# Kaz-K/medical-image-editing

Hardware: AMD Instinct MI355X
Metric: images/sec (train step, 256x256 2D slices) (higher is better)
Workload: dtype f32

## Files before the change

### medical-image-editing_amd/csrc/conv_wino64.hip

```cpp
#include "common.h"
#include "conv_common.h"
#include "mfma_util.h"
#include "wino_common.h"

extern int g_wino_mode;

namespace {

struct W64Args {
    const float* x;
    const float* u;
    const float* bias;
    float* y;
    int N, H, W, Cin, Cout;
    int tilesY, tilesX, nsp;
    int ntn, nch;
    int kt;
    int relu;
    unsigned nbx, nbu, nby;
    float* stats;
    const float* mask;
    const float* mr;
    int in_relu;
    float* y2;
    int split, pool0;
    int c1;
    unsigned nby2;
    unsigned img_px, rowb_px, rpx, ppx;
    int n_sh, n_m;
};

constexpr int W6_KPH = wino::KPH;
template <int RW, int MBW, int NW = 8> struct W64Geo {
    static_assert(MBW == 1 || (MBW == 2 && RW == 32), "two M blocks per wave: 32-wide regions only");
    static_assert(NW == 8 || (NW == 4 && RW == 32), "four-wave workgroups: 32-wide regions only");
    static constexpr int NMB = NW / 2;
    static constexpr int NBW = 4 / MBW;
    static constexpr int NCO = 16 * NBW;
    static constexpr int TR = RW == 32 ? 2 * MBW * NMB : 16;
    static constexpr int HR = TR + 2, HWV = RW + 2;
    static constexpr int HWS = RW == 32 ? 34 : 24;
    static constexpr int HBUF = HR * HWS * W6_KPH;
    static constexpr int UBUF = 16 * NCO * 8;
    static constexpr int EXF = 2048 * NW;
    static_assert(EXF >= UBUF, "U buffer 1 lives in the exchange area");
    static constexpr size_t LDS_FLOATS = 2 * HBUF + UBUF + EXF + 2 * NMB * NCO * 2;
};
constexpr int W6_LS = 4;
constexpr int W6_CP = 26;
constexpr int W6_CP1 = 26;
constexpr int W6_PB = 33, W6_CB = 58;

template <int RW, int MBW, int EPI, int NW = 8>
__global__ void __launch_bounds__(64 * NW, 8 / NW) k_conv_wino64(W64Args a) {
    constexpr bool MASK = EPI >= 1 && EPI <= 3;
    using G = W64Geo<RW, MBW, NW>;
    constexpr int NT = 64 * NW, NMB = G::NMB, NBW = G::NBW, NCO = G::NCO;
    constexpr int HWS = G::HWS, HWV = G::HWV, HBUF = G::HBUF, UBUF = G::UBUF;
    using Halo = wino::HaloStager<NT, G::HR, HWV, HWS, wino::PitchedPix>;
    constexpr int LH = Halo::LH;
    constexpr int LU = 512 * NBW / NT;
    constexpr int CP = MBW == 1 ? W6_CP1 : W6_CP;
    constexpr int CPMAX = MBW == 1 ? 64 : 32;
    constexpr bool ONE_PHASE = 1 + (LH + LU) * W6_LS <= CP && CP + LH + LU <= CPMAX;
    constexpr int LUA = ONE_PHASE ? LU : LU / 2;
    static_assert(1 + (LH + LUA) * W6_LS <= CP && CP + LH + LUA <= CPMAX, "prefetch slots fit the first half of an item");
    static_assert(ONE_PHASE || (LU == 2 * LUA && W6_PB + LUA * W6_LS <= W6_CB && W6_CB + LUA <= 64), "second U phase fits the second half");

    extern __shared__ __attribute__((aligned(16))) float smem[];
    float* Hs = smem;
    float* Us = smem + 2 * HBUF;
    float* Ex = Us + UBUF;
    float* Rs = Ex + G::EXF;

    const int tid = threadIdx.x, lane = tid & 63;
    const int wv = __builtin_amdgcn_readfirstlane(tid >> 6);
    const int mb = wv & (NMB - 1), h = wv / NMB;
    const int H = a.H, W = a.W, Cin = a.Cin, Cout = a.Cout;
    const __amdgpu_buffer_rsrc_t rsx = make_rsrc(a.x, a.nbx), rsu = make_rsrc(a.u, a.nbu), rsy = make_rsrc(a.y, a.nby);
    const __amdgpu_buffer_rsrc_t rsm = make_rsrc((EPI == 1 || EPI == 3) ? a.mask : a.y, a.nby);
    const __amdgpu_buffer_rsrc_t rsr = make_rsrc(EPI == 3 ? a.mr : a.y, EPI == 3 ? (unsigned)((size_t)a.N * a.Cout * 8) : a.nby);
    const __amdgpu_buffer_rsrc_t rsy2 = make_rsrc(EPI == 4 ? a.y2 : a.y, EPI == 4 ? a.nby2 : a.nby);

    const int nch = a.nch;
    const wino::RegionRun run = wino::region_run(a.ntn, a.kt, a.nsp);
    const int co_base = run.tile_n * NCO;
    const int my_tiles = run.my_tiles;
    if (my_tiles <= 0) return;

    const int c4 = tid & 1;
    const wino::PitchedPix pixel = {a.img_px, a.rowb_px, a.rpx, a.ppx, a.n_sh, a.n_m};
    Halo hs;
    hs.init(tid, pixel);
    auto region_offsets = [&](int n, int tx, int ty) { hs.region_offsets(n, ty * G::TR - 1, tx * RW - 1, H, W, Cin); };
    const int u_n = (tid >> 1) & (NCO - 1);
    const unsigned u_voff = (((unsigned)(tid >> 1) / NCO * Cout + co_base + u_n) * 8u + c4 * 4) * 4u;
    const unsigned u_jstride = (unsigned)(NT / 2 / NCO) * Cout * 32u;
    const unsigned u_cstride = 16u * Cout * 32u;
    const int u_lds = (tid >> 1) * 8 + ((c4 ^ ((u_n >> 3) & 1)) * 4);

    float4 ru[LUA];
    auto issue_h = [&](int j, int chunk) { hs.issue_h(rsx, j, chunk); };
    auto commit_h = [&](int j, float* Hb) { hs.commit_h(j, Hb); };
    auto issue_u = [&](int j, int chunk) {
        u32x4 v = __builtin_amdgcn_raw_buffer_load_b128(rsu, (int)u_voff, (int)(chunk * u_cstride + j * u_jstride), 0);
        unsigned a0 = v[0], a1 = v[1], a2 = v[2], a3 = v[3];
        float4& r = ru[j % LUA];
        r.x = __uint_as_float(a0); r.y = __uint_as_float(a1); r.z = __uint_as_float(a2); r.w = __uint_as_float(a3);
    };
    auto commit_u = [&](int j, float* Ub) { *(float4*)&Ub[u_lds + j * (NT * 4)] = ru[j % LUA]; };

    int cn, ctx, cty, ch = 0;
    region_start(run.sp0, a.tilesY, a.tilesX, cn, ctx, cty);
    auto advance = [&](int& n, int& tx, int& ty, int& c) {
        const int adv = c + 1 == nch ? 1 : 0;
        c = adv ? 0 : c + 1;
        region_step(adv, a.tilesY, a.tilesX, n, tx, ty);
    };
    int n1 = cn, tx1 = ctx, ty1 = cty, ch1 = 0;
    advance(n1, tx1, ty1, ch1);
    int n2 = n1, tx2 = tx1, ty2 = ty1, ch2 = ch1;
    advance(n2, tx2, ty2, ch2);
    auto shift = [&]() {
        cn = n1; ctx = tx1; cty = ty1; ch = ch1;
        n1 = n2; tx1 = tx2; ty1 = ty2; ch1 = ch2;
        advance(n2, tx2, ty2, ch2);
    };

    const int m = lane & 15, q = lane >> 4;
    const int rA = h ? 3 : 0, rB = h ? 2 : 1, rC = h ? 1 : 2;
    const int prow = RW == 32 ? 2 * MBW * mb : 2 * (2 * mb + (m >> 3)), pcol = RW == 32 ? 2 * m : 2 * (m & 7);
    constexpr int MBW_STEP = 2 * HWS * W6_KPH;
    const int a_A = opaque(((prow + rA) * HWS + pcol) * W6_KPH + 2 * q);
    const int a_B = opaque(((prow + rB) * HWS + pcol) * W6_KPH + 2 * q);
    const int a_C = opaque(((prow + rC) * HWS + pcol) * W6_KPH + 2 * q);
    const int b_swz = ((q >> 1) ^ (m >> 3)) * 4 + (q & 1) * 2;
    const int b_0 = opaque(((h ? 3 : 0) * 4 * NCO + m) * 8 + b_swz);
    const int b_1 = opaque(((h ? 2 : 1) * 4 * NCO + m) * 8 + b_swz);
    const float sg = opaque_f(h ? -1.f : 1.f), mone = opaque_f(-1.f);

    f32x4 acc[8][MBW][NBW];
    f32x2 bf[2][NBW];
    f32x2 dcol[2][3];
    float e[2][2][4];
    float v[2][MBW][2][8];

    auto read_col = [&](const float* Hb, int w, int c) {
        const float* Hc = Hb + w * MBW_STEP + c * W6_KPH;
        dcol[c & 1][0] = *(const f32x2*)&Hc[a_A];
        dcol[c & 1][1] = *(const f32x2*)&Hc[a_B];
        dcol[c & 1][2] = *(const f32x2*)&Hc[a_C];
    };
    auto xform_op = [&](int par, int w, int o) {
        if (o < 16) {
            const int c = o >> 2, k = o & 3, t = k >> 1;
            const float dA = dcol[c & 1][0][t], dB = dcol[c & 1][1][t], dC = dcol[c & 1][2][t];
            if ((k & 1) == 0) e[t][0][c] = __builtin_fmaf(mone, dC, dA);
            else e[t][1][c] = __builtin_fmaf(sg, dC, dB);
        } else {
            const int k = o - 16, lr = k >> 3, t = (k >> 2) & 1, cc = k & 3;
            const float e0 = e[t][lr][0], e1 = e[t][lr][1], e2 = e[t][lr][2], e3 = e[t][lr][3];
            v[par][w][t][lr * 4 + cc] = wino::bt_row_plain(cc, e0, e1, e2, e3);
        }
    };
    auto xform_slot = [&](const float* Hn, int par, int p) {
        constexpr int NOPS = 32 * MBW, P0 = MBW == 1 ? 32 : 4;
        auto op = [&](int g) { xform_op(par, g >> 5, g & 31); };
        auto rd = [&](int g) {
            if ((g & 31) < 16 && ((g & 31) & 3) == 0) read_col(Hn, g >> 5, (g & 31) >> 2);
        };
        if (p + 3 - P0 >= 0 && p + 3 - P0 < NOPS) rd(p + 3 - P0);
        if (p - P0 >= 0 && p - P0 < NOPS && p < 64) {
            const int g = p - P0;
            if (P0 + NOPS <= 64 || g < NOPS - 2 * (P0 + NOPS - 64)) op(g);
            else { const int d = g - (NOPS - 2 * (P0 + NOPS - 64)); op(NOPS - 2 * (P0 + NOPS - 64) + 2 * d); op(NOPS - 2 * (P0 + NOPS - 64) + 2 * d + 1); }
        }
    };

    region_offsets(cn, ctx, cty);
#pragma unroll
    for (int j = 0; j < LH; ++j) issue_h(j, 0);
#pragma unroll
    for (int j = 0; j < LUA; ++j) issue_u(j, 0);
#pragma unroll
    for (int j = 0; j < LH; ++j) commit_h(j, Hs);
#pragma unroll
    for (int j = 0; j < LUA; ++j) commit_u(j, Us);
#pragma unroll
    for (int j = LUA; j < LU; ++j) issue_u(j, 0);
#pragma unroll
    for (int j = LUA; j < LU; ++j) commit_u(j, Us);
    region_offsets(n1, tx1, ty1);
#pragma unroll
    for (int j = 0; j < LH; ++j) issue_h(j, ch1);
#pragma unroll
    for (int j = 0; j < LH; ++j) commit_h(j, Hs + HBUF);
    __syncthreads();
#pragma unroll
    for (int w = 0; w < MBW; ++w)
#pragma unroll
        for (int o = 0; o < 32; ++o) {
            if (o < 16 && (o & 3) == 0) read_col(Hs, w, o >> 2);
            xform_op(0, w, o);
        }
    __syncthreads();
    region_offsets(n2, tx2, ty2);

    float bvv[NBW / 2];
#pragma unroll
    for (int i = 0; i < NBW / 2; ++i) bvv[i] = a.bias ? a.bias[co_base + (h * (NBW / 2) + i) * 16 + m] : 0.f;
    const float lo = a.relu ? 0.f : -__builtin_inff();
    const bool plain = a.bias == nullptr && !a.relu;
    int spar = 0;

    auto body = [&](auto PAR, auto FIRST) {
        constexpr int par = decltype(PAR)::value;
        constexpr bool first = decltype(FIRST)::value;
        const float* Uc = Us + par * UBUF;
        const float* Hn = Hs + (par ^ 1) * HBUF;
        float* Hw = Hs + par * HBUF;
        float* Uw = Us + (par ^ 1) * UBUF;
        auto ldb = [&](int l, int nb) {
            bf[l & 1][nb] = *(const f32x2*)&Uc[(l < 4 ? b_0 : b_1) + ((l & 3) * NCO + nb * 16) * 8];
        };
        auto slot = [&](int p) {
            if (p >= 1 && p < 1 + LH * W6_LS && (p - 1) % W6_LS == 0) issue_h((p - 1) / W6_LS, ch2);
            if (p >= CP && p < CP + LH) commit_h(p - CP, Hw);
            if (p >= 1 + LH * W6_LS && p < 1 + (LH + LUA) * W6_LS && (p - 1) % W6_LS == 0) issue_u((p - 1) / W6_LS - LH, ch1);
            if (p >= CP + LH && p < CP + LH + LUA) commit_u(p - CP - LH, Uw);
            if (!ONE_PHASE) {
                if (p >= W6_PB && p < W6_PB + LUA * W6_LS && (p - W6_PB) % W6_LS == 0) issue_u(LUA + (p - W6_PB) / W6_LS, ch1);
                if (p >= W6_CB && p < W6_CB + LUA) commit_u(LUA + p - W6_CB, Uw);
            }
            xform_slot(Hn, par ^ 1, p);
        };
#pragma unroll
        for (int nb = 0; nb < NBW; ++nb) { ldb(0, nb); __builtin_amdgcn_sched_barrier(0); }
        const f32x4 zero4 = {0.f, 0.f, 0.f, 0.f};
        if (first) {
#pragma unroll
            for (int p = 0; p < 8; ++p) slot(p);
#pragma unroll
            for (int w = 0; w < MBW; ++w)
#pragma unroll
                for (int nb = 0; nb < NBW; ++nb) acc[7][w][nb] = zero4;
        } else {
#pragma unroll
            for (int j = 0; j < 8; ++j) {
                const int w = j / (2 * NBW), k = (j / NBW) & 1, nb = j % NBW;
                acc[7][w][nb] = MFMA16(v[par ^ 1][w][k][7], k == 0 ? bf[1][nb].x : bf[1][nb].y, acc[7][w][nb]);
                slot(j);
                __builtin_amdgcn_sched_barrier(0);
            }
        }
#pragma unroll
        for (int l = 0; l < 7; ++l) {
#pragma unroll
            for (int j = 0; j < 8; ++j) {
                const int w = j / (2 * NBW), k = (j / NBW) & 1, nb = j % NBW;
                if (j < NBW) ldb(l + 1, nb);
                acc[l][w][nb] = MFMA16(v[par][w][k][l], k == 0 ? bf[l & 1][nb].x : bf[l & 1][nb].y, (first && k == 0) ? zero4 : acc[l][w][nb]);
                slot(8 + l * 8 + j);
                __builtin_amdgcn_sched_barrier(0);
            }
        }
    };
    auto flush = [&]() {
#pragma unroll
        for (int j = 0; j < 8; ++j) {
            const int w = j / (2 * NBW), k = (j / NBW) & 1, nb = j % NBW;
            acc[7][w][nb] = MFMA16(v[1][w][k][7], k == 0 ? bf[1][nb].x : bf[1][nb].y, acc[7][w][nb]);
            __builtin_amdgcn_sched_barrier(0);
        }
    };

    auto partial = [&](auto HH, int w, int nb, int r, float* yv) {
        constexpr int hh = decltype(HH)::value;
        float p0[4], p1[4];
#pragma unroll
        for (int j = 0; j < 4; ++j) {
            const float l0 = acc[j][w][nb][r], l1 = acc[4 + j][w][nb][r];
            if (hh == 0) { p0[j] = l0 + l1; p1[j] = l1; }
            else { p0[j] = l1; p1[j] = l0 - l1; }
        }
        yv[0] = (p0[0] + p0[1]) + p0[2];
        yv[1] = (p0[1] - p0[2]) - p0[3];
        yv[2] = (p1[0] + p1[1]) + p1[2];
        yv[3] = (p1[1] - p1[2]) - p1[3];
    };
    auto epi_send = [&](auto HH) {
        constexpr int hh = decltype(HH)::value;
        float* Xo = Ex + (((mb * 2 + (hh ^ 1)) * 8) * 64 + lane) * 4;
#pragma unroll
        for (int w = 0; w < MBW; ++w)
#pragma unroll
            for (int i = 0; i < NBW / 2; ++i)
#pragma unroll
                for (int r = 0; r < 4; ++r) {
                    float yv[4];
                    partial(HH, w, (hh ^ 1) * (NBW / 2) + i, r, yv);
                    float4 o;
                    o.x = yv[0]; o.y = yv[1]; o.z = yv[2]; o.w = yv[3];
                    *(float4*)&Xo[((w * (NBW / 2) + i) * 4 + r) * 256] = o;
                }
    };
    auto epi_finish = [&](auto HH) {
        constexpr int hh = decltype(HH)::value;
        const float* Xi = Ex + (((mb * 2 + hh) * 8) * 64 + lane) * 4;
        float st1[NBW / 2], st2[NBW / 2];
#pragma unroll
        for (int w = 0; w < MBW; ++w) {
            const int yrow0 = cty * G::TR + (RW == 32 ? 2 * (MBW * mb + w) : 2 * (2 * mb + (q >> 1)));
            const int xcol0 = ctx * RW + (RW == 32 ? 8 * q : 8 * (q & 1));
#pragma unroll
            for (int i = 0; i < NBW / 2; ++i) {
                float yv[16];
                const int co0 = co_base + (hh * (NBW / 2) + i) * 16;
                const unsigned co = (unsigned)(co0 + m);
                const bool part0 = EPI == 4 && co0 < a.split;
                const bool pooled = part0 && a.pool0;
                const unsigned cs = EPI != 4 ? (unsigned)Cout : (unsigned)(part0 ? a.split : a.c1);
                const unsigned cc = EPI != 4 ? co : (part0 ? co : co - (unsigned)a.split);
                int voffs[2];
#pragma unroll
                for (int aa = 0; aa < 2; ++aa) {
                    const int yy = yrow0 + aa;
                    const unsigned base = (pixel.base(cn) + (unsigned)yy * a.rpx + (unsigned)xcol0 * a.ppx) * cs + cc;
                    voffs[aa] = (int)sel_u32(yy < H, base * 4u, 0xFFFFFFFFu);
                }
                float mk[16];
                if (MASK) {
#pragma unroll
                    for (int aa = 0; aa < 2; ++aa)
#pragma unroll
                        for (int r = 0; r < 4; ++r)
#pragma unroll
                            for (int b = 0; b < 2; ++b)
                                mk[r * 4 + aa * 2 + b] = __uint_as_float(__builtin_amdgcn_raw_buffer_load_b32(rsm, voffs[aa], (2 * r + b) * (int)a.ppx * Cout * 4, 0));
                }
#pragma unroll
                for (int r = 0; r < 4; ++r) {
                    float own[4];
                    partial(HH, w, hh * (NBW / 2) + i, r, own);
                    const float4 o = *(const float4*)&Xi[((w * (NBW / 2) + i) * 4 + r) * 256];
                    if (plain) {
                        yv[r * 4 + 0] = own[0] + o.x; yv[r * 4 + 1] = own[1] + o.y;
                        yv[r * 4 + 2] = own[2] + o.z; yv[r * 4 + 3] = own[3] + o.w;
                    } else {
                        yv[r * 4 + 0] = fmaxf((own[0] + o.x) + bvv[i], lo);
                        yv[r * 4 + 1] = fmaxf((own[1] + o.y) + bvv[i], lo);
                        yv[r * 4 + 2] = fmaxf((own[2] + o.z) + bvv[i], lo);
                        yv[r * 4 + 3] = fmaxf((own[3] + o.w) + bvv[i], lo);
                    }
                }
                if (EPI == 1) {
#pragma unroll
                    for (int k = 0; k < 16; ++k) yv[k] = mk[k] > 0.f ? yv[k] : 0.f;
                } else if (EPI == 2) {
#pragma unroll
                    for (int k = 0; k < 16; ++k) yv[k] = mk[k] + yv[k];
                } else if (EPI == 3) {
                    const unsigned mo = ((unsigned)(cn >> a.n_sh) * (unsigned)Cout + co) * 8u;
                    const float mean = __uint_as_float(__builtin_amdgcn_raw_buffer_load_b32(rsr, (int)mo, 0, 0));
                    const float rstd = __uint_as_float(__builtin_amdgcn_raw_buffer_load_b32(rsr, (int)mo, 4, 0));
                    float s1 = 0.f, s2 = 0.f;
#pragma unroll
                    for (int k = 0; k < 16; ++k) {
                        const float xh = (mk[k] - mean) * rstd;
                        const float gm = (a.in_relu && !(xh > 0.f)) ? 0.f : yv[k];
                        s1 += gm;
                        s2 = __builtin_fmaf(gm, xh, s2);
                    }
                    s1 += __shfl_xor(s1, 16, 64); s2 += __shfl_xor(s2, 16, 64);
                    s1 += __shfl_xor(s1, 32, 64); s2 += __shfl_xor(s2, 32, 64);
                    if (w == 0) { st1[i] = s1; st2[i] = s2; }
                    else { st1[i] += s1; st2[i] += s2; }
                }
                if (EPI == 4 && !part0 && co0 - a.split >= a.c1) {
                } else if (EPI == 4 && pooled) {
                    const unsigned base = (((unsigned)cn * (unsigned)(H >> 1) + (unsigned)(yrow0 >> 1)) * (unsigned)(W >> 1) + (unsigned)(xcol0 >> 1)) * cs + cc;
                    const int voff = (int)sel_u32(yrow0 < H, base * 4u, 0xFFFFFFFFu);
#pragma unroll
                    for (int r = 0; r < 4; ++r) {
                        const float t = (yv[r * 4 + 0] + yv[r * 4 + 1]) + (yv[r * 4 + 2] + yv[r * 4 + 3]);
                        __builtin_amdgcn_raw_buffer_store_b32(__float_as_uint(t), rsy, voff, r * (int)cs * 4, 0);
                    }
                } else {
#pragma unroll
                    for (int aa = 0; aa < 2; ++aa) {
                        const int voff = voffs[aa];
#pragma unroll
                        for (int r = 0; r < 4; ++r)
#pragma unroll
                            for (int b = 0; b < 2; ++b)
                                __builtin_amdgcn_raw_buffer_store_b32(__float_as_uint(yv[r * 4 + aa * 2 + b]), (EPI == 4 && !part0) ? rsy2 : rsy, voff,
                                                                      (2 * r + b) * (int)(a.ppx * cs) * 4, 0);
                    }
                }
                if (EPI != 3 && a.stats) {
                    float t1, t2;
                    lane_stats<16>(yv, t1, t2);
                    stat_merge_eq(t1, t2, __shfl_xor(t1, 16, 64), __shfl_xor(t2, 16, 64), 1.f / 32.f);
                    stat_merge_eq(t1, t2, __shfl_xor(t1, 32, 64), __shfl_xor(t2, 32, 64), 1.f / 64.f);
                    if (w == 0) { st1[i] = t1; st2[i] = t2; }
                    else stat_merge_eq(st1[i], st2[i], t1, t2, 1.f / 128.f);
                }
            }
        }
        if (a.stats && lane < 16) {
#pragma unroll
            for (int i = 0; i < NBW / 2; ++i) {
                float* R = Rs + spar * (NMB * NCO * 2) + (mb * NCO + (hh * (NBW / 2) + i) * 16 + lane) * 2;
                R[0] = st1[i];
                R[1] = st2[i];
            }
        }
    };
    auto fold_stats = [&]() {
        if (!a.stats) return;
        if (tid < NCO) {
            const float* R = Rs + spar * (NMB * NCO * 2) + tid * 2;
            float s1 = R[0], s2 = R[1];
            constexpr float PW = 64.f * MBW;
            if (EPI == 3) {
#pragma unroll
                for (int r = 1; r < NMB; ++r) { s1 += R[r * NCO * 2]; s2 += R[r * NCO * 2 + 1]; }
            } else {
#pragma unroll
                for (int r = 1; r < NMB; ++r) stat_merge(s1, s2, PW * r, R[r * NCO * 2], R[r * NCO * 2 + 1], PW);
            }
            const int t = (cn * a.tilesX + ctx) * a.tilesY + cty;
            float* o = a.stats + ((size_t)t * Cout + co_base + tid) * 2;
            o[0] = s1;
            o[1] = s2;
        }
        spar ^= 1;
    };

    using wino::P0;
    using wino::P1;
    for (int reg = 0; reg < my_tiles; ++reg) {
        body(P0{}, std::true_type{});
        __syncthreads();
        shift();
        body(P1{}, std::false_type{});
        __syncthreads();
        for (int c = 2; c < nch; c += 2) {
            shift();
            if (ch2 == 0) region_offsets(n2, tx2, ty2);
            body(P0{}, std::false_type{});
            __syncthreads();
            shift();
            body(P1{}, std::false_type{});
            __syncthreads();
        }
        flush();
        if (h == 0) epi_send(P0{}); else epi_send(P1{});
        __syncthreads();
        if (h == 0) epi_finish(P0{}); else epi_finish(P1{});
        __syncthreads();
        fold_stats();
        shift();
        if (ch2 == 0) region_offsets(n2, tx2, ty2);
    }
}

}

static int wino64_shape(int Cin, int Cout, int W) {
    if (Cin % 16 != 0) return 0;
    if (Cout % 64 == 0) return 1;
    return (Cout % 32 == 0 && W % 32 == 0) ? 2 : 0;
}
static int wino64_waves(int shape) { return shape == 2 ? 4 : 8; }
bool conv_wino64_ok(int Cin, int Cout, int W) { return wino64_shape(Cin, Cout, W) != 0; }
int conv_wino64_stat_tiles(int Cin, int Cout, int H, int W) {
    const int shape = wino64_shape(Cin, Cout, W);
    const int rw = W % 32 == 0 ? 32 : 16, tr = rw == 32 ? shape * wino64_waves(shape) : 16;
    return tr > 0 && H % tr == 0 ? (H / tr) * (W / rw) : 0;
}

template <int RW, int MBW, int EPI, int NW = 8>
static int launch_wino64(W64Args& a, hipStream_t st) {
    using G = W64Geo<RW, MBW, NW>;
    constexpr size_t lds = G::LDS_FLOATS * sizeof(float);
    static_assert(lds * (8 / NW) <= 160 * 1024, "buffers do not fit the 160 KB LDS");
    if (int rc = lds_opt_in<k_conv_wino64<RW, MBW, EPI, NW>>((int)lds, "conv_wino64")) return rc;
    a.tilesY = ceil_div(a.H, G::TR); a.tilesX = a.W / RW; a.nsp = a.N * a.tilesY * a.tilesX;
    a.ntn = a.Cout / G::NCO;
    a.kt = conv_region_runs(a.nsp, a.ntn, 8 / NW);
    k_conv_wino64<RW, MBW, EPI, NW><<<ceil_div(a.nsp, a.kt) * a.ntn, 64 * NW, lds, st>>>(a);
    VQW_LAUNCH_CHECK("conv_wino64");
    return VQW_OK;
}

bool conv_wino64_dil2_ok(int Cin, int Cout, int H, int W) {
    return H % 2 == 0 && W % 64 == 0 && wino64_shape(Cin, Cout, W / 2) != 0;
}
int conv_wino64_fwd(const float* x, const float* u, const float* bias, float* y, int N, int H, int W, int Cin, int Cout, int relu,
                    hipStream_t st, float* stats, const float* mask, int accumulate, const float* in_mr, int in_relu, int dil) {
    W64Args a;
    const long P = (long)N * H * W;
    a.img_px = (unsigned)(H * W); a.rowb_px = 0; a.rpx = (unsigned)W; a.ppx = 1; a.n_sh = 0; a.n_m = 0;
    if (dil == 2) {
        a.rowb_px = (unsigned)W; a.rpx = 2u * (unsigned)W; a.ppx = 2; a.n_sh = 2; a.n_m = 1;
        N *= 4; H /= 2; W /= 2;
    }
    a.y2 = nullptr; a.split = 0; a.pool0 = 0; a.c1 = 0; a.nby2 = 0;
    a.x = x; a.u = u; a.bias = bias; a.y = y; a.mask = mask; a.mr = in_mr; a.in_relu = in_relu;
    a.N = N; a.H = H; a.W = W; a.Cin = Cin; a.Cout = Cout;
    a.nch = Cin / 8;
    a.relu = relu;
    a.stats = stats;
    a.nbx = (unsigned)(P * Cin * 4);
    a.nbu = (unsigned)(16L * Cout * Cin * 4);
    a.nby = (unsigned)(P * Cout * 4);
    const int shape = wino64_shape(Cin, Cout, W);
    if (in_mr) {
        if (shape == 2) return launch_wino64<32, 2, 3, 4>(a, st);
        if (W % 32 == 0) return launch_wino64<32, 1, 3>(a, st);
        return launch_wino64<16, 1, 3>(a, st);
    }
    if (mask) {
        if (shape == 2) return launch_wino64<32, 2, 1, 4>(a, st);
        if (W % 32 == 0) return launch_wino64<32, 1, 1>(a, st);
        return launch_wino64<16, 1, 1>(a, st);
    }
    if (accumulate) {
        if (shape == 2) return launch_wino64<32, 2, 2, 4>(a, st);
        if (W % 32 == 0) return launch_wino64<32, 1, 2>(a, st);
        return launch_wino64<16, 1, 2>(a, st);
    }
    if (shape == 2) return launch_wino64<32, 2, 0, 4>(a, st);
    if (W % 32 == 0) return launch_wino64<32, 1, 0>(a, st);
    return launch_wino64<16, 1, 0>(a, st);
}

bool conv_wino64_split_ok(int Cin, int Cout, int split, int pool0, int N, int H, int W, int c1) {
    if (c1 < 0 || c1 % 16 != 0 || split + c1 > Cout) return false;
    if (!conv_wino64_ok(Cin, Cout, W) || g_wino_mode != 0 || split <= 0 || split >= Cout || split % 16 != 0) return false;
    if (pool0 && (H % 2 != 0)) return false;
    return (long)N * H * W * (Cin > Cout ? Cin : Cout) * 4 <= 0xFFFFFFE0L;
}
int conv_wino64_fwd_split(const float* x, const float* u, const float* bias, float* y0, float* y1, int N, int H, int W, int Cin, int Cout,
                          int split, int pool0, int relu, hipStream_t st, int c1) {
    if (c1 <= 0) c1 = Cout - split;
    W64Args a;
    a.img_px = (unsigned)(H * W); a.rowb_px = 0; a.rpx = (unsigned)W; a.ppx = 1; a.n_sh = 0; a.n_m = 0;
    a.x = x; a.u = u; a.bias = bias; a.y = y0; a.y2 = y1; a.mask = nullptr; a.mr = nullptr; a.in_relu = 0;
    a.split = split; a.pool0 = pool0; a.c1 = c1;
    a.N = N; a.H = H; a.W = W; a.Cin = Cin; a.Cout = Cout;
    a.nch = Cin / 8;
    a.relu = relu;
    a.stats = nullptr;
    const long P = (long)N * H * W;
    a.nbx = (unsigned)(P * Cin * 4);
    a.nbu = (unsigned)(16L * Cout * Cin * 4);
    a.nby = (unsigned)((pool0 ? P / 4 : P) * split * 4);
    a.nby2 = (unsigned)(P * c1 * 4);
    const int shape = wino64_shape(Cin, Cout, W);
    if (shape == 2) return launch_wino64<32, 2, 4, 4>(a, st);
    if (W % 32 == 0) return launch_wino64<32, 1, 4>(a, st);
    return launch_wino64<16, 1, 4>(a, st);
}

namespace {

struct W64WgArgs {
    const float* x;
    const float* dy;
    float* part;
    float* bias_part;
    int N, H, W, Cin, Cout;
    int tilesY, tilesX, nsp;
    int n_ci_b, nblk, kt;
    unsigned nbx, nbd;
    const float* x1;
    int C0, up0;
    unsigned nbx1;
    unsigned img_px, rowb_px, rpx, ppx;
    int n_sh, n_m;
};

constexpr int W6_WLS = 2;
constexpr int WG_XP = 40;
template <int RW, int MB> struct WgGeo {
    static_assert((MB == 4 && (RW == 32 || RW == 16)) || (MB == 2 && RW == 32), "the 16-wide region needs the dense rows of the 64-cout form");
    static constexpr int DP = 16 * MB + 8;
    static constexpr int TRP = RW == 32 ? 4 : 8;
    static constexpr int XW = RW + 2, XR = TRP + 2, XPIX = XR * XW;
    static constexpr int DBUF = 128 * DP, XBUF = XPIX * WG_XP;
    static constexpr size_t LDS_BYTES = (size_t)2 * (DBUF + XBUF) * sizeof(float);
    static_assert(LDS_BYTES <= 160 * 1024 && LDS_BYTES >= 64 * 1024, "tiles fit the LDS; the fold needs 64 KB");
};

template <int RW, int MB>
__global__ void __launch_bounds__(512, 1) k_conv_wino_wgrad_blk(W64WgArgs a) {
    using G = WgGeo<RW, MB>;
    constexpr int NT = 512, DP = G::DP, DBUF = G::DBUF, XBUF = G::XBUF, XW = G::XW;
    constexpr int XF = G::XPIX * 8;
    constexpr int LX = (XF + NT - 1) / NT;
    constexpr int QD = 4 * MB;
    constexpr int DPX = NT / QD, LD = MB;
    constexpr int NP = 8 * MB;
    constexpr bool PITCH = MB == 2;
    extern __shared__ __attribute__((aligned(16))) float smem[];

    const int tid = threadIdx.x, lane = tid & 63;
    const int wv = __builtin_amdgcn_readfirstlane(tid >> 6);
    const int r = wv & 3, kh = wv >> 2;
    const int H = a.H, W = a.W, Cin = a.Cin, Cout = a.Cout;
    const int lb = xcd_remap(blockIdx.x, gridDim.x);
    const int blk = lb % a.nblk, sblk = lb / a.nblk;
    const int co_base = (blk / a.n_ci_b) * (16 * MB), ci_base = (blk % a.n_ci_b) * 32;
    const int sp0 = sblk * a.kt;
    const int my_tiles = min(a.kt, a.nsp - sp0);
    const bool do_bias = a.bias_part != nullptr && ci_base == 0;
    const unsigned rpx = PITCH ? a.rpx : (unsigned)W, ppx = PITCH ? a.ppx : 1u;

    const int d_px = tid / QD;
    const unsigned d_fix = (((unsigned)(d_px / RW) * rpx + (unsigned)(d_px % RW) * ppx) * Cout + co_base + (tid % QD) * 4) * 4u;
    const unsigned d_jstride = (unsigned)(DPX / RW) * rpx * Cout * 4u;
    const int d_lds = d_px * DP + (tid % QD) * 4;
    const bool x_s1 = ci_base >= a.C0;
    const bool x_up = !x_s1 && a.up0;
    const float* x_ptr = x_s1 ? a.x1 : a.x;
    const int x_cs = x_s1 ? Cin - a.C0 : a.C0, x_cb = x_s1 ? ci_base - a.C0 : ci_base;
    const int x_w = x_up ? W >> 1 : W, x_h = x_up ? H >> 1 : H;
    const long x_nb = x_s1 ? (long)a.nbx1 : (long)a.nbx;
    const unsigned x_rpx = x_up ? (unsigned)x_w : rpx, x_ppx = x_up ? 1u : ppx;
    unsigned x_fix[LX];
    int x_lds[LX];
    unsigned x_bits = 0;
#pragma unroll
    for (int j = 0; j < LX; ++j) {
        int f = tid + j * NT;
        if (f >= XF) f -= XF;
        const int hp = f >> 3, hy = hp / XW, hx = hp - hy * XW;
        x_fix[j] = (((unsigned)(x_up ? (hy + 1) >> 1 : hy) * x_rpx + (unsigned)(x_up ? (hx + 1) >> 1 : hx) * x_ppx) * x_cs + x_cb + (tid & 7) * 4) * 4u;
        x_lds[j] = 2 * DBUF + hp * WG_XP + (tid & 7) * 4;
        x_bits |= (unsigned)((hy == 0 ? 1 : 0) | (hy == G::XR - 1 ? 2 : 0) | (hx == 0 ? 4 : 0) | (hx == XW - 1 ? 8 : 0)) << (4 * j);
    }
    float4 rd[LD], rx[LX];
    float4 bsum;
    bsum.x = bsum.y = bsum.z = bsum.w = 0.f;
    __amdgpu_buffer_rsrc_t rsd, rsx;
    unsigned x_edges = 0;
    auto region_setup = [&](int n, int tx, int ty) {
        const int y0 = ty * G::TRP, x0 = tx * RW;
        long dpix;
        if constexpr (PITCH) {
            const long nbase = (long)(n >> a.n_sh) * a.img_px + (long)((n >> 1) & a.n_m) * a.rowb_px + (n & a.n_m);
            dpix = nbase + (long)y0 * a.rpx + (long)x0 * a.ppx;
        } else {
            dpix = ((long)n * H + y0) * W + x0;
        }
        const long doff = dpix * Cout * 4;
        rsd = __builtin_amdgcn_make_buffer_rsrc((void*)((const char*)a.dy + doff), 0, (int)(unsigned)((long)a.nbd - doff), 0x00020000);
        const long xpix = x_up ? ((long)n * x_h + (y0 >> 1) - 1) * x_w + (x0 >> 1) - 1
                               : PITCH ? dpix - (long)a.rpx - (long)a.ppx : dpix - W - 1;
        const long xoff = xpix * x_cs * 4;
        const long xleft = x_nb - xoff;
        rsx = __builtin_amdgcn_make_buffer_rsrc((void*)((const char*)x_ptr + xoff), 0, (int)(unsigned)(xleft > 0xFFFFFFF0L ? 0xFFFFFFF0L : xleft), 0x00020000);
        x_edges = ((y0 == 0 ? 1u : 0u) | (y0 + G::TRP == H ? 2u : 0u) | (x0 == 0 ? 4u : 0u) | (x0 + RW == W ? 8u : 0u)) * 0x1111u;
    };
    auto issue_d = [&](int j) { rd[j] = buf_ld4(rsd, d_fix, j * d_jstride); };
    auto issue_x = [&](int j) {
        const unsigned vo = (x_bits & x_edges & (0xFu << (4 * j))) ? 0xFFFFFFFFu : x_fix[j];
        rx[j] = buf_ld4(rsx, vo, 0);
    };
    float once_v = 1.f;
    auto commit_d = [&](int j, int buf) {
        *(float4*)&smem[d_lds + buf * DBUF + j * DPX * DP] = rd[j];
        if (do_bias) {
            bsum.x = __builtin_fmaf(once_v, rd[j].x, bsum.x); bsum.y = __builtin_fmaf(once_v, rd[j].y, bsum.y);
            bsum.z = __builtin_fmaf(once_v, rd[j].z, bsum.z); bsum.w = __builtin_fmaf(once_v, rd[j].w, bsum.w);
        }
    };
    auto commit_x = [&](int j, int buf) { *(float4*)&smem[x_lds[j] + buf * XBUF] = rx[j]; };

    const int idx = lane & 15, k = lane >> 4;
    const int aF = r == 3 ? 1 : 0, aS = r == 0 ? 0 : 1;
    const int trow0 = RW == 32 ? kh : 2 * kh;
    const int a_F = opaque(((2 * trow0 + aF) * RW + 2 * k) * DP + idx);
    const int a_S = opaque(((2 * trow0 + aS) * RW + 2 * k) * DP + idx);
    const int iA = r == 0 ? 0 : r == 2 ? 2 : 1, iB = r == 0 ? 2 : r == 1 ? 2 : r == 2 ? 1 : 3;
    const int x_A = opaque(2 * DBUF + ((2 * trow0 + iA) * XW + 2 * k) * WG_XP + idx);
    const int x_B = opaque(2 * DBUF + ((2 * trow0 + iB) * XW + 2 * k) * WG_XP + idx);
    const float sA = opaque_f((r == 1) ? 1.f : (r == 2) ? -1.f : 0.f), sB = opaque_f((r == 1) ? 1.f : -1.f);
    auto s_px_d = [](int s) { return RW == 32 ? 8 * s : 2 * (s >> 1) * 16 + 8 * (s & 1); };
    auto s_px_x = [](int s) { return RW == 32 ? 8 * s : 2 * (s >> 1) * XW + 8 * (s & 1); };

    f32x4 acc[4][MB][2];
#pragma unroll
    for (int c = 0; c < 4; ++c)
#pragma unroll
        for (int mb = 0; mb < MB; ++mb)
#pragma unroll
            for (int nb = 0; nb < 2; ++nb)
#pragma unroll
                for (int q = 0; q < 4; ++q) acc[c][mb][nb][q] = 0.f;
    float dm[2][MB][4];
    float vv[2][2][4];
    float ra[2][4], rb[2][8];

    auto rd_grp = [&](int nbuf, int s, int g, int i) {
        if (g < MB) {
            const int o = nbuf * DBUF + s_px_d(s) * DP + g * 16 + (i & 1) * DP;
            ra[g & 1][i] = i < 2 ? smem[a_F + o] : smem[a_S + o];
        } else {
            const int o = nbuf * XBUF + s_px_x(s) * WG_XP + (g - MB) * 16 + (i & 3) * WG_XP;
            rb[g & 1][i] = i < 4 ? smem[x_A + o] : smem[x_B + o];
        }
    };
    auto op_grp = [&](int set, int g, int i) {
        if (g < MB) {
            float* d = dm[set][g];
            const float* q = ra[g & 1];
            if (i == 0) d[0] = __builtin_fmaf(sA, q[2], q[0]);
            if (i == 1) d[3] = __builtin_fmaf(sA, q[3], q[1]);
            if (i == 2) d[1] = d[0] + d[3];
            if (i == 3) d[2] = d[0] - d[3];
        } else {
            float* o = vv[set][g - MB];
            float* q = rb[g & 1];
            if (i < 4) q[i] = __builtin_fmaf(sB, q[4 + i], q[i]);
            if (i == 4) o[0] = q[0] - q[2];
            if (i == 5) o[1] = q[1] + q[2];
            if (i == 6) o[2] = q[2] - q[1];
            if (i == 7) o[3] = q[1] - q[3];
        }
    };
    auto build_slot = [&](int nbuf, int s, int set, int p) {
        if constexpr (MB == 4) {
            if (p < 4) rd_grp(nbuf, s, 0, p);
            else if (p < 16) { op_grp(set, (p - 4) >> 2, (p - 4) & 3); rd_grp(nbuf, s, ((p - 4) >> 2) + 1, (p - 4) & 3); }
            else if (p < 20) { op_grp(set, 3, p - 16); rd_grp(nbuf, s, 4, 2 * (p - 16)); rd_grp(nbuf, s, 4, 2 * (p - 16) + 1); }
            else if (p < 28) { op_grp(set, 4, p - 20); rd_grp(nbuf, s, 5, p - 20); }
            else { op_grp(set, 5, 2 * (p - 28)); op_grp(set, 5, 2 * (p - 28) + 1); }
        } else {
            auto rd2 = [&](int g, int i0) { rd_grp(nbuf, s, g, i0); rd_grp(nbuf, s, g, i0 + 1); };
            auto op2 = [&](int g, int i0) { op_grp(set, g, i0); op_grp(set, g, i0 + 1); };
            if (p == 0) rd2(0, 0);
            else if (p == 1) rd2(0, 2);
            else if (p == 2) rd2(1, 0);
            else if (p == 3) { op2(0, 0); rd2(1, 2); }
            else if (p == 4) { op2(0, 2); rd2(2, 0); }
            else if (p == 5) { op2(1, 0); rd2(2, 2); }
            else if (p == 6) { op2(1, 2); rd2(2, 4); }
            else if (p == 7) rd2(2, 6);
            else if (p < 12) { op2(2, 2 * (p - 8)); rd2(3, 2 * (p - 8)); }
            else op2(3, 2 * (p - 12));
        }
    };

    int cn, ctx, cty;
    region_start(sp0, a.tilesY, a.tilesX, cn, ctx, cty);
    if (my_tiles > 0) {
        region_setup(cn, ctx, cty);
#pragma unroll
        for (int j = 0; j < LD; ++j) issue_d(j);
#pragma unroll
        for (int j = 0; j < LX; ++j) issue_x(j);
#pragma unroll
        for (int j = 0; j < LD; ++j) commit_d(j, 0);
#pragma unroll
        for (int j = 0; j < LX; ++j) commit_x(j, 0);
        __syncthreads();
#pragma unroll
        for (int p = 0; p < NP; ++p) build_slot(0, 0, 0, p);
    }
    int ln = cn, ltx = ctx, lty = cty, lcount = 0;
    auto load_advance = [&]() {
        if (lcount + 1 < my_tiles) { region_next(a.tilesY, a.tilesX, ln, ltx, lty); ++lcount; once_v = 1.f; } else once_v = 0.f;
        region_setup(ln, ltx, lty);
    };
    if (my_tiles > 0) {
        load_advance();
#pragma unroll
        for (int j = 0; j < LD; ++j) issue_d(j);
    }

    auto phase = [&](auto SET, auto SNEXT, auto NBUF, auto DBUFW, auto LOADS) {
        constexpr int set = decltype(SET)::value, sn = decltype(SNEXT)::value, nbuf = decltype(NBUF)::value;
        constexpr int wbuf = decltype(DBUFW)::value, loads = decltype(LOADS)::value;
#pragma unroll
        for (int c = 0; c < 4; ++c)
#pragma unroll
            for (int mb = 0; mb < MB; ++mb)
#pragma unroll
                for (int nb = 0; nb < 2; ++nb) {
                    const int p = c * 2 * MB + mb * 2 + nb;
                    acc[c][mb][nb] = MFMA16(dm[set][mb][c], vv[set][nb][c], acc[c][mb][nb]);
                    build_slot(nbuf, sn, set ^ 1, p);
                    if (loads == 0 && p >= 8 && p < 8 + LD) commit_d(p - 8, wbuf);
                    if (loads == 1 && p >= 2 && p < 2 + W6_WLS * LX && (p - 2) % W6_WLS == 0) issue_x((p - 2) / W6_WLS);
                    if (loads == 2 && p >= 8 && p < 8 + LX) commit_x(p - 8, wbuf);
                    if (loads == 3 && p >= 2 && p < 2 + W6_WLS * LD && (p - 2) % W6_WLS == 0) issue_d((p - 2) / W6_WLS);
                    __builtin_amdgcn_sched_barrier(0);
                }
    };
    using I0 = std::integral_constant<int, 0>;
    using I1 = std::integral_constant<int, 1>;
    using I2 = std::integral_constant<int, 2>;
    using I3 = std::integral_constant<int, 3>;
    auto region = [&](auto BUF) {
        constexpr int b = decltype(BUF)::value;
        using B = std::integral_constant<int, b>;
        using NB = std::integral_constant<int, b ^ 1>;
        phase(I0{}, I1{}, B{}, NB{}, I0{});
        phase(I1{}, I2{}, B{}, NB{}, I1{});
        phase(I0{}, I3{}, B{}, NB{}, I2{});
        __syncthreads();
        load_advance();
        phase(I1{}, I0{}, NB{}, B{}, I3{});
    };
    for (int g = 0; g < my_tiles; g += 2) {
        region(I0{});
        if (g + 1 < my_tiles) region(I1{});
    }

    __syncthreads();
    float* red = smem;
    if (do_bias) {
        *(float4*)&red[tid * 4] = bsum;
        __syncthreads();
        if (tid < 16 * MB) {
            const int cq = tid >> 2, comp = tid & 3;
            float sum = 0.f;
            for (int i = 0; i < DPX; ++i) sum += red[(i * QD + cq) * 4 + comp];
            a.bias_part[(size_t)sblk * Cout + co_base + tid] = sum;
        }
        __syncthreads();
    }
    int fold_w = ((kh * 4 + r) * 4 * 16 + 4 * (lane >> 4)) * 32 + idx, fold_r = tid;
    asm volatile("" : "+v"(fold_w), "+v"(fold_r));
#pragma unroll
    for (int mb = 0; mb < MB; ++mb) {
#pragma unroll
        for (int c = 0; c < 4; ++c)
#pragma unroll
            for (int nb = 0; nb < 2; ++nb)
#pragma unroll
                for (int q = 0; q < 4; ++q)
                    red[fold_w + c * 512 + q * 32 + nb * 16] = acc[c][mb][nb][q];
        __syncthreads();
        {
            const int e = fold_r;
            float tcol[3][4];
#pragma unroll
            for (int c = 0; c < 4; ++c) {
                float u[4];
#pragma unroll
                for (int rr = 0; rr < 4; ++rr) {
                    const float t = red[((0 * 4 + rr) * 4 + c) * 512 + e] + red[((1 * 4 + rr) * 4 + c) * 512 + e];
                    u[rr] = ((rr == 3) != (c == 3)) ? -t : t;
                }
                tcol[0][c] = u[0] + 0.5f * (u[1] + u[2]);
                tcol[1][c] = 0.5f * (u[1] - u[2]);
                tcol[2][c] = u[3] + 0.5f * (u[1] + u[2]);
            }
            const int co = co_base + mb * 16 + (tid >> 5), ci = ci_base + (tid & 31);
            float* o = a.part + (size_t)sblk * Cout * 9 * Cin + ((size_t)co * 9) * Cin + ci;
#pragma unroll
            for (int ky = 0; ky < 3; ++ky) {
                const float t0 = tcol[ky][0], t1 = tcol[ky][1], t2 = tcol[ky][2], t3 = tcol[ky][3];
                o[(ky * 3 + 0) * Cin] = t0 + 0.5f * (t1 + t2);
                o[(ky * 3 + 1) * Cin] = 0.5f * (t1 - t2);
                o[(ky * 3 + 2) * Cin] = t3 + 0.5f * (t1 + t2);
            }
        }
        __syncthreads();
    }
}

}

static int wgrad_blk_mb(int C0, int C1, int up0, int Cout, int H, int W) {
    if (C1 == 0 ? (up0 || C0 % 32 != 0)
                : (C0 % 32 != 0 || C1 % 32 != 0 || (up0 && (H % 2 != 0 || W % 2 != 0)))) return 0;
    if (Cout % 64 == 0) return (W % 16 == 0 && H % (W % 32 == 0 ? 4 : 8) == 0) ? 4 : 0;
    return (Cout % 32 == 0 && W % 32 == 0 && H % 4 == 0) ? 2 : 0;
}
bool conv_wino_blk_wgrad_ok(int C0, int C1, int up0, int Cout, int H, int W) { return wgrad_blk_mb(C0, C1, up0, Cout, H, W) != 0; }
bool conv_wino_blk_wgrad_dil2_ok(int C0, int Cout, int H, int W) {
    return H % 2 == 0 && W % 2 == 0 && wgrad_blk_mb(C0, 0, 0, Cout, H / 2, W / 2) == 2;
}
int conv_wino_blk_wgrad_blocks(int Cin, int Cout, int N, int H, int W, int max_slabs, int* kt_out) {
    const int rw = W % 32 == 0 ? 32 : 16;
    return conv_slab_split(N * (H / (128 / rw)) * (W / rw), (Cout / (Cout % 64 == 0 ? 64 : 32)) * (Cin / 32), max_slabs, kt_out);
}
template <int RW, int MB>
static int launch_wgrad_blk(const W64WgArgs& a, int nsb, hipStream_t st) {
    if (int rc = lds_opt_in<k_conv_wino_wgrad_blk<RW, MB>>(160 * 1024, "conv_wino_blk_wgrad")) return rc;
    k_conv_wino_wgrad_blk<RW, MB><<<a.nblk * nsb, 512, WgGeo<RW, MB>::LDS_BYTES, st>>>(a);
    VQW_LAUNCH_CHECK("conv_wino_blk_wgrad");
    return VQW_OK;
}
int conv_wino_blk_wgrad(const ConvIn& in, const float* dy, float* ws, float* bpart, int N, int H, int W, int Cin, int Cout, int nsb, int kt,
                        hipStream_t st, int dil) {
    const long P = (long)N * H * W;
    W64WgArgs a;
    a.dy = dy; a.part = ws; a.bias_part = bpart;
    a.Cin = Cin; a.Cout = Cout;
    a.x = in.src0; a.x1 = in.C1 ? in.src1 : in.src0; a.C0 = in.C0; a.up0 = in.C1 ? in.up0 : 0;
    a.nbx = (unsigned)((a.up0 ? P / 4 : P) * in.C0 * 4);
    a.nbx1 = (unsigned)(P * in.C1 * 4);
    a.nbd = (unsigned)(P * Cout * 4);
    a.img_px = (unsigned)(H * W); a.rowb_px = 0; a.rpx = (unsigned)W; a.ppx = 1; a.n_sh = 0; a.n_m = 0;
    if (dil == 2) {
        a.rowb_px = (unsigned)W; a.rpx = 2u * (unsigned)W; a.ppx = 2; a.n_sh = 2; a.n_m = 1;
        N *= 4; H /= 2; W /= 2;
    }
    a.N = N; a.H = H; a.W = W;
    const int rw = W % 32 == 0 ? 32 : 16, mb = Cout % 64 == 0 ? 4 : 2;
    a.tilesY = H / (128 / rw); a.tilesX = W / rw; a.nsp = N * a.tilesY * a.tilesX;
    a.n_ci_b = Cin / 32; a.nblk = (Cout / (16 * mb)) * a.n_ci_b; a.kt = kt;
    if (mb == 2) return launch_wgrad_blk<32, 2>(a, nsb, st);
    return rw == 32 ? launch_wgrad_blk<32, 4>(a, nsb, st) : launch_wgrad_blk<16, 4>(a, nsb, st);
}
```

### medical-image-editing_amd/csrc/wino_common.h

```cpp
#pragma once
#include "mfma_util.h"
#include <type_traits>

namespace wino {

using P0 = std::integral_constant<int, 0>;
using P1 = std::integral_constant<int, 1>;

struct RegionRun {
    int tile_n, sp0, my_tiles;
};
__device__ __forceinline__ RegionRun region_run(int ntn, int kt, int nsp) {
    const int lb = xcd_remap(blockIdx.x, gridDim.x);
    RegionRun r;
    r.tile_n = lb % ntn;
    r.sp0 = (lb / ntn) * kt;
    r.my_tiles = min(kt, nsp - r.sp0);
    return r;
}

template <class Args>
struct ItemCursor {
    const Args& a;
    int cn, ctx, cty, ch;
    int n1, tx1, ty1, ch1;
    int n2, tx2, ty2, ch2;
    __device__ __forceinline__ void advance(int& n, int& tx, int& ty, int& c) const {
        const int adv = c + 1 == a.nch ? 1 : 0;
        c = adv ? 0 : c + 1;
        region_step(adv, a.tilesY, a.tilesX, n, tx, ty);
    }
    __device__ __forceinline__ ItemCursor(const Args& a_, int sp0) : a(a_) {
        region_start(sp0, a.tilesY, a.tilesX, cn, ctx, cty);
        ch = 0;
        n1 = cn; tx1 = ctx; ty1 = cty; ch1 = 0;
        advance(n1, tx1, ty1, ch1);
        n2 = n1; tx2 = tx1; ty2 = ty1; ch2 = ch1;
        advance(n2, tx2, ty2, ch2);
    }
    __device__ __forceinline__ void shift() {
        cn = n1; ctx = tx1; cty = ty1; ch = ch1;
        n1 = n2; tx1 = tx2; ty1 = ty2; ch1 = ch2;
        advance(n2, tx2, ty2, ch2);
    }
};

template <class Cursor, class Body, class Offsets, class Epilogue>
__device__ __forceinline__ void region_loop(int my_tiles, int nch, Cursor& it, Body&& body, Offsets&& offsets, Epilogue&& epilogue) {
    for (int reg = 0; reg < my_tiles; ++reg) {
        body(P0{}, std::true_type{});
        __syncthreads();
        it.shift();
        body(P1{}, std::false_type{});
        __syncthreads();
        for (int c = 2; c < nch; c += 2) {
            it.shift();
            if (it.ch2 == 0) offsets(it.n2, it.tx2, it.ty2);
            body(P0{}, std::false_type{});
            __syncthreads();
            it.shift();
            body(P1{}, std::false_type{});
            __syncthreads();
        }
        epilogue();
        it.shift();
        if (it.ch2 == 0) offsets(it.n2, it.tx2, it.ty2);
    }
}

struct DensePix {
    unsigned H, W;
    __device__ __forceinline__ unsigned operator()(int n, int yy, int xx) const { return ((unsigned)n * H + (unsigned)yy) * W + (unsigned)xx; }
};
struct PitchedPix {
    unsigned img_px, rowb_px, rpx, ppx;
    int n_sh, n_m;
    __device__ __forceinline__ unsigned base(int n) const {
        return (unsigned)(n >> n_sh) * img_px + (unsigned)((n >> 1) & n_m) * rowb_px + (unsigned)(n & n_m);
    }
    __device__ __forceinline__ unsigned operator()(int n, int yy, int xx) const { return base(n) + (unsigned)yy * rpx + (unsigned)xx * ppx; }
};

constexpr int KPH = 10;

template <int NT, int HR, int HWV, int HWS, class Pix>
struct HaloStager {
    static constexpr int HF = HR * HWV * 2;
    static constexpr int LH = (HF + NT - 1) / NT;
    static_assert(HF > (LH - 1) * NT && HF >= NT, "every halo slot but the last is full");
    Pix pix;
    int tid, c4;
    int h_lds[LH];
    unsigned h_voff[LH];
    float4 rh[LH];
    __device__ __forceinline__ void halo_pixel(int j, int& hy, int& hx) const {
        int f = tid + j * NT;
        if (f >= HF) f -= HF;
        const int hp = f >> 1;
        hy = hp / HWV;
        hx = hp - hy * HWV;
    }
    __device__ __forceinline__ void init(int tid_, const Pix& pix_) {
        tid = tid_; c4 = tid_ & 1; pix = pix_;
#pragma unroll
        for (int j = 0; j < LH; ++j) {
            int hy, hx;
            halo_pixel(j, hy, hx);
            h_lds[j] = (hy * HWS + hx) * KPH + c4 * 4;
        }
    }
    __device__ __forceinline__ void region_offsets(int n, int y0, int x0, int H, int W, int C) {
#pragma unroll
        for (int j = 0; j < LH; ++j) {
            int hy, hx;
            halo_pixel(j, hy, hx);
            const int yy = y0 + hy, xx = x0 + hx;
            const bool ok = ((unsigned)yy < (unsigned)H) & ((unsigned)xx < (unsigned)W);
            h_voff[j] = sel_u32(ok, pix(n, yy, xx) * (unsigned)C * 4u + (unsigned)c4 * 16u, 0xFFFFFFFFu);
        }
    }
    __device__ __forceinline__ void issue_h(__amdgpu_buffer_rsrc_t rs, int j, int chunk) { rh[j] = buf_ld4(rs, h_voff[j], chunk * 32); }
    __device__ __forceinline__ void commit_h(int j, float* Hb) {
        float* p = Hb + h_lds[j];
        f32x2 lo, hi;
        lo.x = rh[j].x; lo.y = rh[j].y; hi.x = rh[j].z; hi.y = rh[j].w;
        *(f32x2*)p = lo;
        *(f32x2*)(p + 2) = hi;
    }
};

__device__ __forceinline__ float bt_row(int r, float d0, float d1, float d2, float d3, float pone, float mone) {
    return r == 0 ? __builtin_fmaf(mone, d2, d0) : r == 1 ? __builtin_fmaf(pone, d2, d1) : r == 2 ? __builtin_fmaf(mone, d1, d2) : __builtin_fmaf(mone, d3, d1);
}
__device__ __forceinline__ float bt_row_plain(int r, float d0, float d1, float d2, float d3) {
    return r == 0 ? d0 - d2 : r == 1 ? d1 + d2 : r == 2 ? d2 - d1 : d1 - d3;
}

__device__ __forceinline__ void weight_transform(const double g[3][3], double u[4][4]) {
    double t[4][3];
    for (int kx = 0; kx < 3; ++kx) {
        t[0][kx] = g[0][kx];
        t[1][kx] = 0.5 * (g[0][kx] + g[1][kx] + g[2][kx]);
        t[2][kx] = 0.5 * (g[0][kx] - g[1][kx] + g[2][kx]);
        t[3][kx] = g[2][kx];
    }
    for (int i = 0; i < 4; ++i) {
        u[i][0] = t[i][0];
        u[i][1] = 0.5 * (t[i][0] + t[i][1] + t[i][2]);
        u[i][2] = 0.5 * (t[i][0] - t[i][1] + t[i][2]);
        u[i][3] = t[i][2];
    }
}

}
```

Measured before the change: 353.5.

## Load Winograd weight tiles straight into LDS with buffer-load-to-LDS DMA

```diff
diff --git a/medical-image-editing_amd/csrc/conv_wino64.hip b/medical-image-editing_amd/csrc/conv_wino64.hip
--- a/medical-image-editing_amd/csrc/conv_wino64.hip
+++ b/medical-image-editing_amd/csrc/conv_wino64.hip
@@ -47,9 +47,8 @@
     static constexpr size_t LDS_FLOATS = 2 * HBUF + UBUF + EXF + 2 * NMB * NCO * 2;
 };
 constexpr int W6_LS = 4;
-constexpr int W6_CP = 26;
-constexpr int W6_CP1 = 26;
-constexpr int W6_PB = 33, W6_CB = 58;
+constexpr int W6_ULS = 2;
+constexpr int W6_CP = 48;
 
 template <int RW, int MBW, int EPI, int NW = 8>
 __global__ void __launch_bounds__(64 * NW, 8 / NW) k_conv_wino64(W64Args a) {
@@ -60,12 +59,8 @@
     using Halo = wino::HaloStager<NT, G::HR, HWV, HWS, wino::PitchedPix>;
     constexpr int LH = Halo::LH;
     constexpr int LU = 512 * NBW / NT;
-    constexpr int CP = MBW == 1 ? W6_CP1 : W6_CP;
-    constexpr int CPMAX = MBW == 1 ? 64 : 32;
-    constexpr bool ONE_PHASE = 1 + (LH + LU) * W6_LS <= CP && CP + LH + LU <= CPMAX;
-    constexpr int LUA = ONE_PHASE ? LU : LU / 2;
-    static_assert(1 + (LH + LUA) * W6_LS <= CP && CP + LH + LUA <= CPMAX, "prefetch slots fit the first half of an item");
-    static_assert(ONE_PHASE || (LU == 2 * LUA && W6_PB + LUA * W6_LS <= W6_CB && W6_CB + LUA <= 64), "second U phase fits the second half");
+    constexpr int HP0 = 1 + LU * W6_ULS;
+    static_assert(HP0 + (LH - 1) * W6_LS < W6_CP && W6_CP + LH <= 64, "prefetch slots fit the item");
 
     extern __shared__ __attribute__((aligned(16))) float smem[];
     float* Hs = smem;
@@ -94,21 +89,18 @@
     hs.init(tid, pixel);
     auto region_offsets = [&](int n, int tx, int ty) { hs.region_offsets(n, ty * G::TR - 1, tx * RW - 1, H, W, Cin); };
     const int u_n = (tid >> 1) & (NCO - 1);
-    const unsigned u_voff = (((unsigned)(tid >> 1) / NCO * Cout + co_base + u_n) * 8u + c4 * 4) * 4u;
+    const int u_swz = (u_n >> 3) & 1;
+    const int u_c4 = c4 ^ u_swz;
+    const unsigned u_voff = (((unsigned)(tid >> 1) / NCO * Cout + co_base + u_n) * 8u + u_c4 * 4) * 4u;
     const unsigned u_jstride = (unsigned)(NT / 2 / NCO) * Cout * 32u;
     const unsigned u_cstride = 16u * Cout * 32u;
-    const int u_lds = (tid >> 1) * 8 + ((c4 ^ ((u_n >> 3) & 1)) * 4);
-
-    float4 ru[LUA];
+    const int u_wave = wv * 256;
+
     auto issue_h = [&](int j, int chunk) { hs.issue_h(rsx, j, chunk); };
     auto commit_h = [&](int j, float* Hb) { hs.commit_h(j, Hb); };
-    auto issue_u = [&](int j, int chunk) {
-        u32x4 v = __builtin_amdgcn_raw_buffer_load_b128(rsu, (int)u_voff, (int)(chunk * u_cstride + j * u_jstride), 0);
-        unsigned a0 = v[0], a1 = v[1], a2 = v[2], a3 = v[3];
-        float4& r = ru[j % LUA];
-        r.x = __uint_as_float(a0); r.y = __uint_as_float(a1); r.z = __uint_as_float(a2); r.w = __uint_as_float(a3);
-    };
-    auto commit_u = [&](int j, float* Ub) { *(float4*)&Ub[u_lds + j * (NT * 4)] = ru[j % LUA]; };
+    auto issue_u = [&](int j, int chunk, float* Ub) {
+        wino::buf_ld4_lds(rsu, Ub + u_wave + j * (NT * 4), u_voff, chunk * u_cstride + j * u_jstride);
+    };
 
     int cn, ctx, cty, ch = 0;
     region_start(run.sp0, a.tilesY, a.tilesX, cn, ctx, cty);
@@ -181,20 +173,15 @@
 #pragma unroll
     for (int j = 0; j < LH; ++j) issue_h(j, 0);
 #pragma unroll
-    for (int j = 0; j < LUA; ++j) issue_u(j, 0);
+    for (int j = 0; j < LU; ++j) issue_u(j, 0, Us);
 #pragma unroll
     for (int j = 0; j < LH; ++j) commit_h(j, Hs);
-#pragma unroll
-    for (int j = 0; j < LUA; ++j) commit_u(j, Us);
-#pragma unroll
-    for (int j = LUA; j < LU; ++j) issue_u(j, 0);
-#pragma unroll
-    for (int j = LUA; j < LU; ++j) commit_u(j, Us);
     region_offsets(n1, tx1, ty1);
 #pragma unroll
     for (int j = 0; j < LH; ++j) issue_h(j, ch1);
 #pragma unroll
     for (int j = 0; j < LH; ++j) commit_h(j, Hs + HBUF);
+    wino::dma_wait();
     __syncthreads();
 #pragma unroll
     for (int w = 0; w < MBW; ++w)
@@ -223,15 +210,11 @@
         auto ldb = [&](int l, int nb) {
             bf[l & 1][nb] = *(const f32x2*)&Uc[(l < 4 ? b_0 : b_1) + ((l & 3) * NCO + nb * 16) * 8];
         };
+        static_assert(par == 0 || (par ^ 1) == 0, "a region's last item (odd) loads U into buffer 0: buffer 1 is the epilogue's exchange area");
         auto slot = [&](int p) {
-            if (p >= 1 && p < 1 + LH * W6_LS && (p - 1) % W6_LS == 0) issue_h((p - 1) / W6_LS, ch2);
-            if (p >= CP && p < CP + LH) commit_h(p - CP, Hw);
-            if (p >= 1 + LH * W6_LS && p < 1 + (LH + LUA) * W6_LS && (p - 1) % W6_LS == 0) issue_u((p - 1) / W6_LS - LH, ch1);
-            if (p >= CP + LH && p < CP + LH + LUA) commit_u(p - CP - LH, Uw);
-            if (!ONE_PHASE) {
-                if (p >= W6_PB && p < W6_PB + LUA * W6_LS && (p - W6_PB) % W6_LS == 0) issue_u(LUA + (p - W6_PB) / W6_LS, ch1);
-                if (p >= W6_CB && p < W6_CB + LUA) commit_u(LUA + p - W6_CB, Uw);
-            }
+            if (p >= 1 && p < HP0 && (p - 1) % W6_ULS == 0) issue_u((p - 1) / W6_ULS, ch1, Uw);
+            if (p >= HP0 && p < HP0 + LH * W6_LS && (p - HP0) % W6_LS == 0) issue_h((p - HP0) / W6_LS, ch2);
+            if (p >= W6_CP && p < W6_CP + LH) commit_h(p - W6_CP, Hw);
             xform_slot(Hn, par ^ 1, p);
         };
 #pragma unroll
@@ -439,20 +422,24 @@
 
     using wino::P0;
     using wino::P1;
+    auto item_end = [&]() {
+        wino::dma_wait();
+        __syncthreads();
+    };
     for (int reg = 0; reg < my_tiles; ++reg) {
         body(P0{}, std::true_type{});
-        __syncthreads();
+        item_end();
         shift();
         body(P1{}, std::false_type{});
-        __syncthreads();
+        item_end();
         for (int c = 2; c < nch; c += 2) {
             shift();
             if (ch2 == 0) region_offsets(n2, tx2, ty2);
             body(P0{}, std::false_type{});
-            __syncthreads();
+            item_end();
             shift();
             body(P1{}, std::false_type{});
-            __syncthreads();
+            item_end();
         }
         flush();
         if (h == 0) epi_send(P0{}); else epi_send(P1{});
diff --git a/medical-image-editing_amd/csrc/wino_common.h b/medical-image-editing_amd/csrc/wino_common.h
--- a/medical-image-editing_amd/csrc/wino_common.h
+++ b/medical-image-editing_amd/csrc/wino_common.h
@@ -129,6 +129,11 @@
     }
 };
 
+__device__ __forceinline__ void buf_ld4_lds(__amdgpu_buffer_rsrc_t r, float* lds_wave, unsigned byte_off, unsigned soff) {
+    __builtin_amdgcn_raw_ptr_buffer_load_lds(r, (__attribute__((address_space(3))) void*)lds_wave, 16, (int)byte_off, (int)soff, 0, 0);
+}
+__device__ __forceinline__ void dma_wait() { __builtin_amdgcn_s_waitcnt(0x0F70); }
+
 __device__ __forceinline__ float bt_row(int r, float d0, float d1, float d2, float d3, float pone, float mone) {
     return r == 0 ? __builtin_fmaf(mone, d2, d0) : r == 1 ? __builtin_fmaf(pone, d2, d1) : r == 2 ? __builtin_fmaf(mone, d1, d2) : __builtin_fmaf(mone, d3, d1);
 }
```

Result: faster. 357.2, median of 6 (+1.0%).
